# UCSD-Comp-Imaging/Nerf-Simple

Measured on AMD Instinct MI355X. Metric: ray-samples/sec at 800x800x128, higher is better.
Workload: dtype f16

## Files before the change

### nerf-simple_amd/csrc/mlp16_chain.h

```cpp
#pragma once
#include "nerf_device.h"
#include <utility>

typedef elem_t ex8 __attribute__((ext_vector_type(8)));
typedef elem_t ex2 __attribute__((ext_vector_type(2)));

namespace {

using namespace nerf_layout;

constexpr int NCB = 2;
constexpr int WAVES = 16 / NCB;
constexpr int TILE_PTS = WAVES * 16 * NCB;

template <class P>
__host__ __device__ constexpr int layer_chunks(int L) { return (P::mt(L) + P::tpc(L) - 1) / P::tpc(L); }
template <class P>
__host__ __device__ constexpr int chunk_first(int L) {
    int c = 0;
    for (int i = 0; i < L; ++i) c += layer_chunks<P>(i);
    return c;
}
template <class P>
constexpr int NUM_CHUNKS = chunk_first<P>(P::LAYERS);
template <class P>
__host__ __device__ constexpr int chunk_layer(int cc) {
    int L = 0;
    while (cc >= layer_chunks<P>(L)) { cc -= layer_chunks<P>(L); ++L; }
    return L;
}
template <class P>
__host__ __device__ constexpr int chunk_tiles(int cc) {
    const int L = chunk_layer<P>(cc), C = cc - chunk_first<P>(L);
    const int left = P::mt(L) - C * P::tpc(L);
    return left < P::tpc(L) ? left : P::tpc(L);
}
template <class P>
__host__ __device__ constexpr int chunk_kib(int cc) { return chunk_tiles<P>(cc) * b16_ks(chunk_layer<P>(cc)); }
template <class P>
__host__ __device__ constexpr int chunk_off_kib(int cc) {
    const int L = chunk_layer<P>(cc), C = cc - chunk_first<P>(L);
    return P::layer_off_kib(L) + C * P::tpc(L) * b16_ks(L);
}
template <class P>
__host__ __device__ constexpr int tile_mfmas() {
    int m = 0;
    for (int cc = 0; cc < NUM_CHUNKS<P>; ++cc) m += chunk_kib<P>(cc) * NCB;
    return m;
}

constexpr int LDS_WBUF = 40 * 1024;
constexpr int LDS_BIAS = 0;
constexpr int LDS_W0 = 10 * 1024;
constexpr int LDS_CHAIN_END = LDS_W0 + 2 * LDS_WBUF;
static_assert(B16_BIAS_FLOATS * 4 <= LDS_W0, "bias table");
template <class P>
__host__ __device__ constexpr bool plan_fits() {
    for (int cc = 0; cc < NUM_CHUNKS<P>; ++cc)
        if (chunk_kib<P>(cc) * 1024 > LDS_WBUF) return false;
    return NUM_CHUNKS<P> % 2 == 0;
}

struct Ctx {
    __amdgpu_buffer_rsrc_t wrsrc;
    unsigned wave_goff, lane16;
    unsigned b_wread[2];
    unsigned s_wdst[2];
    unsigned b_bias;
    unsigned b_posx, b_posd;
    int wave, lane;
};

struct WFrag {
    ex8 a[4];
    f32x4 bias0;
};

template <bool RELU>
__device__ __forceinline__ unsigned pack2(float a, float b) {
    const f32x2 v = {a, b};
    const ex2 r = __builtin_convertvector(v, ex2);
    if constexpr (RELU) {
        const s16x2 z = {0, 0};
        return __builtin_bit_cast(unsigned, __builtin_elementwise_max(__builtin_bit_cast(s16x2, r), z));
    } else {
        return __builtin_bit_cast(unsigned, r);
    }
}

template <class P, int CC>
using Stage = ChunkDma<Ctx, (CC + 1) % NUM_CHUNKS<P>, chunk_kib<P>((CC + 1) % NUM_CHUNKS<P>), chunk_off_kib<P>((CC + 1) % NUM_CHUNKS<P>), WAVES>;

template <int L, int Q, int SAVE = 0, class St>
__device__ __forceinline__ void epilogue_piece(int i, const f32x4 (&acc)[NCB][2], ex8 (&dst)[NCB][8], St& st) {
    static_assert(!SAVE || St::Plan::SAVE, "this plan has no training forward");
    constexpr LayerDesc D = layer_desc(L);
    const int cb = i >> 2, j2 = i & 3;
    if constexpr (Q == 0 && L >= 1 && L <= 9) {
        if (j2 == 0) st.bad |= __builtin_amdgcn_classf(acc[cb][0][0], 0x207);
    }
    if constexpr (L == 10) {
        if (j2 == 0) { st.rgb[cb][0] = acc[cb][0][0]; st.rgb[cb][1] = acc[cb][0][1]; st.rgb[cb][2] = acc[cb][0][2]; }
    } else if constexpr (L == 8 && Q == 8) {
        if (j2 == 0) st.sigma[cb] = acc[cb][0][0];
    } else {
        u32x4 w = __builtin_bit_cast(u32x4, dst[cb][Q]);
        w[j2] = pack2<D.relu != 0>(acc[cb][j2 >> 1][2 * (j2 & 1)], acc[cb][j2 >> 1][2 * (j2 & 1) + 1]);
        dst[cb][Q] = __builtin_bit_cast(ex8, w);
        if constexpr (SAVE == 2) {
            constexpr int GS = (L & 1) * 2 + ((Q >> 2) & 1);
            st.amax[GS] = f8_absmax<D.relu == 0>(((Q & 3) == 0 && i == 0) ? 0.f : st.amax[GS], acc[cb][j2 >> 1][2 * (j2 & 1)],
                                                 acc[cb][j2 >> 1][2 * (j2 & 1) + 1]);
            if constexpr ((Q & 3) == 3) {
                if (i == 4 * NCB - 1) {
                    static_assert(NCB == 2, "store_group_f8 takes the two column blocks of a wave");
                    constexpr int Q0 = Q - 3;
                    char* tb = st.acts + (f8_offset_bytes(L, st.P) + st.tile * F8_BLOCK_BYTES);
                    char* sp = st.acts + (f8_scale_offset_bytes(L, st.P) + st.tile * 64);
                    const __amdgpu_buffer_rsrc_t rs = __builtin_amdgcn_make_buffer_rsrc(tb, 0, (int)F8_BLOCK_BYTES, 0x00020000);
                    const __amdgpu_buffer_rsrc_t rss = __builtin_amdgcn_make_buffer_rsrc(sp, 0, 64, 0x00020000);
                    const u32x4 g0[4] = {__builtin_bit_cast(u32x4, dst[0][Q0]), __builtin_bit_cast(u32x4, dst[0][Q0 + 1]),
                                         __builtin_bit_cast(u32x4, dst[0][Q0 + 2]), __builtin_bit_cast(u32x4, dst[0][Q0 + 3])};
                    const u32x4 g1[4] = {__builtin_bit_cast(u32x4, dst[1][Q0]), __builtin_bit_cast(u32x4, dst[1][Q0 + 1]),
                                         __builtin_bit_cast(u32x4, dst[1][Q0 + 2]), w};
                    store_group_f8<2>(rs, st.loff[0], Q0 * 8192, rss, (int)(threadIdx.x & 63), (int)(threadIdx.x >> 6) * 8 + Q0,
                                      g0, g1, st.amax[GS]);
                }
            }
        }
        if constexpr (SAVE) {
            if (SAVE == 1 && j2 == 3) {
                char* tb = st.acts + (act_offset_bytes(L, st.P) + st.tile * ACT_BLOCK_BYTES);
                const __amdgpu_buffer_rsrc_t rs = __builtin_amdgcn_make_buffer_rsrc(tb, 0, (int)ACT_BLOCK_BYTES, 0x00020000);
                store_granule<2>(rs, st.loff[cb], Q * 16384, w);
            }
            if constexpr (D.relu != 0) {
                static_assert(NCB == 2, "mask layout: two column blocks per wave");
                const unsigned wj = w[j2];
                unsigned t;
                asm("v_pk_min_u16 %0, %1, %2" : "=v"(t) : "v"(wj), "s"(0x00010001u));
                const int pos = (Q & 3) * 4 + j2;
                st.mb[cb][Q >> 2] = pos == 0 ? t : ((t << pos) | st.mb[cb][Q >> 2]);
                if (pos == 15) {
                    char* mp = st.acts + (st.mask_tile + ((long long)L * mask_tiles(st.P) * 4 + (cb * 2 + (Q >> 2))) * 2048);
                    *reinterpret_cast<unsigned*>(mp + (unsigned)(threadIdx.x * 4)) = st.mb[cb][Q >> 2];
                }
            }
        }
    }
}

template <int SAVE>
__host__ __device__ constexpr int pair_vmem_ops(int L, int Q) {
    if (!SAVE || L < 0 || L == 10 || (L == 8 && Q == 8)) return 0;
    const int masks = (layer_desc(L).relu != 0 && (Q & 3) == 3) ? NCB : 0;
    return (SAVE == 2 ? ((Q & 3) == 3 ? F8_GROUP + 1 : 0) : NCB) + masks;
}
template <int SAVE>
__host__ __device__ constexpr int pair_mask_ops(int L, int Q) {
    if (!SAVE || L < 0 || L == 10 || (L == 8 && Q == 8)) return 0;
    return (layer_desc(L).relu != 0 && (Q & 3) == 3) ? NCB : 0;
}
template <int SAVE>
__host__ __device__ constexpr int vmem_before_barrier(int L, int PL, int PQ, int pair0, int npair_in, int pend_m0, int pend_per,
                                                      int pair_m0, int mt, int m_limit) {
    int n = 0;
    const int last = 4 * NCB - 1;
    if (PL >= 0) {
        const int masks = pair_mask_ops<SAVE>(PL, PQ), data = pair_vmem_ops<SAVE>(PL, PQ) - masks;
        for (int cb = 0; cb < NCB; ++cb) {
            const int own = 4 * cb + 3;
            if (pend_m0 + own / pend_per < m_limit) n += masks / NCB + (SAVE == 2 ? 0 : data / NCB);
        }
        if (SAVE == 2 && pend_m0 + last / pend_per < m_limit) n += data;
    }
    for (int j = 0; j < npair_in; ++j) {
        const int masks = pair_mask_ops<SAVE>(L, pair0 + j), data = pair_vmem_ops<SAVE>(L, pair0 + j) - masks;
        for (int cb = 0; cb < NCB; ++cb) {
            const int own = 4 * cb + 3;
            if (pair_m0 + j * 2 * mt + own < m_limit) n += masks / NCB + (SAVE == 2 ? 0 : data / NCB);
        }
        if (SAVE == 2 && pair_m0 + j * 2 * mt + last < m_limit) n += data;
    }
    return n;
}
template <int L, int P0, int N, int SAVE, int J = 0, class St>
__device__ __forceinline__ void in_chunk_epilogue(int j, int i, const f32x4 (&acc)[NCB][2], ex8 (&dst)[NCB][8], St& st) {
    if constexpr (J < N) {
        if (j == J) epilogue_piece<L, P0 + J, SAVE>(i, acc, dst, st);
        else in_chunk_epilogue<L, P0, N, SAVE, J + 1>(j, i, acc, dst, st);
    }
}

template <int L, int C, int PL, int PQ, int SAVE, class St>
__device__ __forceinline__ void chunk_step(const Ctx& c, St& st, ex8 (&in)[NCB][8], ex8 (&out)[NCB][8]) {
    using P = typename St::Plan;
    constexpr LayerDesc D = layer_desc(L);
    constexpr int KS_CHAIN = D.chain_k / 32;
    constexpr int KS_EXTRA = D.extra_slots / 32;
    constexpr int KS = KS_CHAIN + KS_EXTRA;
    constexpr int CC = chunk_first<P>(L) + C;
    constexpr int NT = chunk_tiles<P>(CC);
    constexpr int RT0 = C * P::tpc(L);
    constexpr int F = NT * KS;
    constexpr int AHEAD = 4;
    constexpr int BIAS_OFF = LDS_BIAS + (P::bias_off(L) + 16 * RT0) * 4;
    constexpr int MT = NCB * KS;
    constexpr int PEND_M0 = (L == 10) ? 0 : (NT * MT >= 4 * NCB + 4 ? 2 : 0);
    constexpr int PEND_PER = (L == 10) ? 2 : 1;
    constexpr int PAIR0 = RT0 / 2;
    constexpr int NPAIR_IN = NT >= 4 ? NT / 2 - 1 : 0;
    constexpr int PAIR_M0 = 2 * MT + (MT >= 4 * NCB + 2 ? 2 : 0);
    static_assert(NT < 4 || NT % 2 == 0, "whole pairs per chunk");
    static_assert(PL < 0 || PL == L || (PL == 8 && PQ == 8) || NCB * PQ >= PEND_M0 + 4 * NCB / PEND_PER,
                  "pending pair finished too late");
    const unsigned wb = c.b_wread[CC & 1];
    constexpr int NCC = (CC + 1) % NUM_CHUNKS<P>;
    constexpr int NL = chunk_layer<P>(NCC);
    constexpr int NF = chunk_tiles<P>(NCC) * (layer_desc(NL).chain_k / 32 + layer_desc(NL).extra_slots / 32);
    constexpr int NBIAS_OFF = LDS_BIAS + (P::bias_off(NL) + 16 * (NCC - chunk_first<P>(NL)) * P::tpc(NL)) * 4;
    const unsigned nwb = c.b_wread[NCC & 1];
    constexpr int TAIL = 3;
    constexpr int FB = F <= TAIL ? F : F - TAIL;
    constexpr int VMEM_N = vmem_before_barrier<SAVE>(L, PL, PQ, PAIR0, NPAIR_IN, PEND_M0, PEND_PER, PAIR_M0, MT, FB * NCB);
    WFrag& wf = *st.wf;
    auto barrier_and_prefetch = [&]() {
        asm volatile("s_waitcnt lgkmcnt(0)" ::: "memory");
        chunk_barrier<VMEM_N>();
#pragma unroll
        for (int f = 0; f < AHEAD && f < NF; ++f) wf.a[f] = lds_load<ex8>(nwb, f * 1024);
        wf.bias0 = lds_load<f32x4>(c.b_bias, NBIAS_OFF);
        __builtin_amdgcn_sched_barrier(0);
    };

    constexpr int SPREAD = 4;
    constexpr bool DMA_SPREAD = !SAVE && 1 + SPREAD * (Stage<P, CC>::PIECES - 1) + 8 <= FB * NCB;
    if constexpr (!DMA_SPREAD) Stage<P, CC>::issue(c);
    __builtin_amdgcn_sched_barrier(0);

    ex8 a[AHEAD];
#pragma unroll
    for (int f = 0; f < AHEAD && f < F; ++f) a[f] = wf.a[f];
    ex8 bx[NCB][KS_EXTRA > 0 ? KS_EXTRA : 1];
    if constexpr (KS_EXTRA > 0) {
#pragma unroll
        for (int cb = 0; cb < NCB; ++cb)
#pragma unroll
            for (int e = 0; e < KS_EXTRA; ++e) {
                if constexpr (D.extra_kind == 1) bx[cb][e] = lds_load<ex8>(c.b_posx, cb * 2048 + e * 1024);
                else bx[cb][e] = lds_load<ex8>(st.posd_off[cb], e * 1024);
            }
    }
    f32x4 acc[NCB][NT];
    acc[0][0] = wf.bias0;
    for (int cb = 1; cb < NCB; ++cb) acc[cb][0] = acc[0][0];
    __builtin_amdgcn_sched_barrier(0);

    ex8 as_prev = a[0];
    f32x4 c_prev = acc[0][0];
#pragma unroll
    for (int t = 0; t < NT; ++t) {
#pragma unroll
        for (int ks = 0; ks < KS; ++ks) {
            const int f = t * KS + ks;
            if (f == FB) barrier_and_prefetch();
            const ex8 as = a[f % AHEAD];
            if (f + AHEAD < F) a[f % AHEAD] = lds_load<ex8>(wb, (f + AHEAD) * 1024);
            if (t + 1 < NT && ks == KS / 2) {
                acc[0][t + 1 < NT ? t + 1 : 0] = lds_load<f32x4>(c.b_bias, BIAS_OFF + 64 * (t + 1));
                for (int cb = 1; cb < NCB; ++cb) acc[cb][t + 1 < NT ? t + 1 : 0] = acc[0][t + 1 < NT ? t + 1 : 0];
            }
            __builtin_amdgcn_sched_barrier(0);
#pragma unroll
            for (int cb = 0; cb < NCB; ++cb) {
                const int m = f * NCB + cb;
                ex8 bs;
                if (ks < KS_CHAIN) bs = in[cb][ks < KS_CHAIN ? ks : 0];
                else bs = bx[cb][KS_EXTRA > 0 ? (ks - KS_CHAIN < KS_EXTRA ? ks - KS_CHAIN : 0) : 0];
                const f32x4 c_old = acc[cb][t];
                acc[cb][t] = NERF_MFMA(as, bs, c_old, 0, 0, 0);
                asm volatile("" :: "v"(c_prev));
                c_prev = c_old;
                if constexpr (DMA_SPREAD) {
                    if (m % SPREAD == 1 && m / SPREAD < Stage<P, CC>::PIECES) Stage<P, CC>::issue_piece(c, m / SPREAD);
                }
                if constexpr (PL >= 0) {
                    if (m >= PEND_M0 && m < PEND_M0 + 4 * NCB / PEND_PER) {
#pragma unroll
                        for (int k = 0; k < PEND_PER; ++k) {
                            const int i = (m - PEND_M0) * PEND_PER + k;
                            if constexpr (PL == L) epilogue_piece<PL, PQ, SAVE>(i, st.pend, out, st);
                            else epilogue_piece<PL, PQ, SAVE>(i, st.pend, in, st);
                        }
                    }
                }
                if constexpr (NPAIR_IN > 0) {
                    const int j = (m - PAIR_M0) / (2 * MT), pm = (m - PAIR_M0) - j * (2 * MT);
                    if (m >= PAIR_M0 && j < NPAIR_IN && pm < 4 * NCB) {
                        f32x4 pr[NCB][2];
                        for (int q_ = 0; q_ < NCB; ++q_) { pr[q_][0] = acc[q_][2 * j]; pr[q_][1] = acc[q_][2 * j + 1]; }
                        in_chunk_epilogue<L, PAIR0, NPAIR_IN, SAVE>(j, pm, pr, out, st);
                    }
                }
                __builtin_amdgcn_sched_barrier(0);
            }
            asm volatile("" :: "v"(as_prev));
            as_prev = as;
            __builtin_amdgcn_sched_barrier(0);
        }
    }
    asm volatile("" :: "v"(as_prev));
    asm volatile("" :: "v"(c_prev));
#pragma unroll
    for (int cb = 0; cb < NCB; ++cb) {
        st.pend[cb][0] = acc[cb][NT >= 2 ? NT - 2 : 0];
        st.pend[cb][1] = acc[cb][NT - 1];
    }
    if constexpr (FB == F) barrier_and_prefetch();
}

__host__ __device__ constexpr int prev_layer(int L, int C) { return C > 0 ? L : L - 1; }
template <class P>
__host__ __device__ constexpr int prev_pair(int L, int C) {
    return C > 0 ? C * P::tpc(L) / 2 - 1 : (L > 0 ? (L - 1 == 8 ? 8 : P::mt(L - 1) / 2 - 1) : 0);
}

template <int L, int SAVE, class St, int... Cs>
__device__ __forceinline__ void run_layer_seq(const Ctx& c, St& st, ex8 (&in)[NCB][8], ex8 (&out)[NCB][8],
                                              std::integer_sequence<int, Cs...>) {
    using P = typename St::Plan;
    (chunk_step<L, Cs, prev_layer(L, Cs), prev_pair<P>(L, Cs), SAVE>(c, st, in, out), ...);
}
template <int L, int SAVE = 0, class St>
__device__ __forceinline__ void run_layer(const Ctx& c, St& st, ex8 (&in)[NCB][8], ex8 (&out)[NCB][8]) {
    run_layer_seq<L, SAVE>(c, st, in, out, std::make_integer_sequence<int, layer_chunks<typename St::Plan>(L)>{});
}

__device__ __forceinline__ void flag_nonfinite(const Ctx& c, bool bad) {
    if (bad) __builtin_amdgcn_raw_buffer_store_b32(1u, c.wrsrc, (int)(B16_STATUS_OFF + 4 * NERF_STATUS_WORD_NONFINITE), 0, 0);
}

}
```

### nerf-simple_amd/csrc/mlp_bwd_16.hip

```cpp
#include "nerf_device.h"
#include "launchers.h"
#include <utility>

using namespace nerf_layout;

typedef __bf16 ex8 __attribute__((ext_vector_type(8)));
typedef __bf16 ex2 __attribute__((ext_vector_type(2)));
typedef unsigned u32x2 __attribute__((ext_vector_type(2)));

struct BwdArgs {
    const float* d_raw;
    const void* image;
    const char* acts;
    char* dys;
    long long P;
    int store_e4m3;
};

namespace {

constexpr int WAVES = 8;
constexpr int TILE_PTS = WAVES * 32;
constexpr int TPC = 4;

__host__ __device__ constexpr int layer_chunks(int b) { return (bwd_mt(b) + TPC - 1) / TPC; }
__host__ __device__ constexpr int chunk_first(int b) {
    int c = 0;
    for (int i = 0; i < b; ++i) c += layer_chunks(i);
    return c;
}
constexpr int NUM_CHUNKS = chunk_first(NUM_BWD);
__host__ __device__ constexpr int chunk_layer(int cc) {
    int b = 0;
    while (cc >= layer_chunks(b)) { cc -= layer_chunks(b); ++b; }
    return b;
}
__host__ __device__ constexpr int chunk_kib(int cc) { return TPC * bwd_ks(chunk_layer(cc)); }
__host__ __device__ constexpr int chunk_off_kib(int cc) {
    const int b = chunk_layer(cc), C = cc - chunk_first(b);
    return bwd_layer_off_kib(b) + C * TPC * bwd_ks(b);
}

constexpr int LDS_WBUF = 40 * 1024;
constexpr int LDS_W0 = 0;
constexpr int LDS_TOTAL = 2 * LDS_WBUF;
static_assert(NUM_CHUNKS % 2 == 0, "buffer parity must repeat per tile");

static_assert(ACT_TILE_PTS == TILE_PTS && MASK_TILE_PTS == TILE_PTS, "activation blocks and mask tiles are the kernel's tiles");

struct Ctx {
    __amdgpu_buffer_rsrc_t wrsrc;
    unsigned wave_goff, lane16;
    unsigned b_wread[2], s_wdst[2];
    int wave, lane;
};

struct State {
    ex8 X[2][8], Y[2][8];
    f32x4 pend[2][2];
    u32x4 mk[2];
    long long mask_tile;
    ex8 bx_rgb[2], bx_sig[2];
    const char* acts;
    char* dys;
    long long P, tile;
    int loff[2];
    float amax[4];
};

__device__ __forceinline__ unsigned pack2(float a, float b) {
    const f32x2 v = {a, b};
    return __builtin_bit_cast(unsigned, __builtin_convertvector(v, ex2));
}

template <int CC>
using Stage = ChunkDma<Ctx, (CC + 1) % NUM_CHUNKS, chunk_kib((CC + 1) % NUM_CHUNKS), chunk_off_kib((CC + 1) % NUM_CHUNKS), WAVES>;

template <int A>
__device__ __forceinline__ void load_mask(const State& st, u32x4& m) {
    const char* mp = st.acts + (st.mask_tile + (long long)A * mask_tiles(st.P) * 8192);
#pragma unroll
    for (int d = 0; d < 4; ++d) m[d] = *reinterpret_cast<const unsigned*>(mp + d * 2048 + (unsigned)(threadIdx.x * 4));
}

template <int B, int Q, bool F8>
__device__ __forceinline__ void epilogue_piece(int i, const f32x4 (&acc)[2][2], ex8 (&dst)[2][8], State& st) {
    constexpr BwdDesc D = bwd_desc(B);
    constexpr int LOUT = 9 - B;
    const int cb = i >> 2, j2 = i & 3;
    float v0 = acc[cb][j2 >> 1][2 * (j2 & 1)], v1 = acc[cb][j2 >> 1][2 * (j2 & 1) + 1];
    if constexpr (D.mask_act >= 0) {
        const unsigned mw = st.mk[B & 1][cb * 2 + (Q >> 2)];
        const int pos = (Q & 3) * 4 + j2;
        v0 = __builtin_bit_cast(float, __builtin_bit_cast(int, v0) & ((int)(mw << (31 - pos)) >> 31));
        v1 = __builtin_bit_cast(float, __builtin_bit_cast(int, v1) & ((int)(mw << (15 - pos)) >> 31));
    }
    u32x4 w = __builtin_bit_cast(u32x4, dst[cb][Q]);
    w[j2] = pack2(v0, v1);
    dst[cb][Q] = __builtin_bit_cast(ex8, w);
    if constexpr (F8) {
        constexpr int GS = (B & 1) * 2 + ((Q >> 2) & 1);
        st.amax[GS] = f8_absmax<true>(((Q & 3) == 0 && i == 0) ? 0.f : st.amax[GS], v0, v1);
        if constexpr ((Q & 3) == 3) {
            if (i == 7) {
                constexpr int Q0 = Q - 3;
                char* tb = st.dys + (f8_offset_bytes(LOUT, st.P) + st.tile * F8_BLOCK_BYTES);
                char* sp = st.dys + (f8_scale_offset_bytes(LOUT, st.P) + st.tile * 64);
                const __amdgpu_buffer_rsrc_t rs = __builtin_amdgcn_make_buffer_rsrc(tb, 0, (int)F8_BLOCK_BYTES, 0x00020000);
                const __amdgpu_buffer_rsrc_t rss = __builtin_amdgcn_make_buffer_rsrc(sp, 0, 64, 0x00020000);
                const u32x4 g0[4] = {__builtin_bit_cast(u32x4, dst[0][Q0]), __builtin_bit_cast(u32x4, dst[0][Q0 + 1]),
                                     __builtin_bit_cast(u32x4, dst[0][Q0 + 2]), __builtin_bit_cast(u32x4, dst[0][Q0 + 3])};
                const u32x4 g1[4] = {__builtin_bit_cast(u32x4, dst[1][Q0]), __builtin_bit_cast(u32x4, dst[1][Q0 + 1]),
                                     __builtin_bit_cast(u32x4, dst[1][Q0 + 2]), w};
                store_group_f8<2>(rs, st.loff[0], Q0 * 8192, rss, (int)(threadIdx.x & 63), (int)(threadIdx.x >> 6) * 8 + Q0, g0, g1,
                                  st.amax[GS]);
            }
        }
    } else if (j2 == 3) {
        char* tb = st.dys + (act_offset_bytes(LOUT, st.P) + st.tile * ACT_BLOCK_BYTES);
        const __amdgpu_buffer_rsrc_t rs = __builtin_amdgcn_make_buffer_rsrc(tb, 0, (int)ACT_BLOCK_BYTES, 0x00020000);
        store_granule<2>(rs, st.loff[cb], Q * 16384, w);
    }
}

template <int B, int C, int PB, int PQ, bool F8>
__device__ __forceinline__ void chunk_step(const Ctx& c, State& st, ex8 (&in)[2][8], ex8 (&out)[2][8]) {
    constexpr BwdDesc D = bwd_desc(B);
    constexpr int KS_CHAIN = D.chain_k / 32;
    constexpr int KS = KS_CHAIN + D.extra;
    constexpr int CC = chunk_first(B) + C;
    constexpr int NT = TPC;
    constexpr int F = NT * KS;
    constexpr int AHEAD = 4;
    constexpr int MT = 2 * KS;
    constexpr int TOTAL_M = NT * MT;
    constexpr bool PEND_EARLY = TOTAL_M < 24 || (PB != B && PB >= 0 && 2 * PQ < 12);
    constexpr int PEND_PER = PEND_EARLY ? 2 : 1;
    constexpr int PEND_M0 = PEND_EARLY ? 0 : 2;
    static_assert(PB < 0 || PB == B || 2 * PQ >= PEND_M0 + 8 / PEND_PER, "pending pair finished too late");
    constexpr int PAIR_M0 = TOTAL_M >= 24 ? 2 * MT + 2 : 2 * MT;
    constexpr int PAIR_PER = (TOTAL_M - PAIR_M0) >= 8 ? 1 : 2;
    const unsigned wb = c.b_wread[CC & 1];
    static_assert(bwd_mt(B) % TPC == 0, "row tiles per backward layer");

    Stage<CC>::issue(c);
    __builtin_amdgcn_sched_barrier(0);

    ex8 a[AHEAD];
#pragma unroll
    for (int f = 0; f < AHEAD && f < F; ++f) a[f] = lds_load<ex8>(wb, f * 1024);
    if constexpr (C == 1 && B + 1 < NUM_BWD) {
        if constexpr (bwd_desc(B + 1).mask_act >= 0) load_mask<bwd_desc(B + 1).mask_act>(st, st.mk[(B + 1) & 1]);
    }
    static_assert(layer_chunks(B) >= 2, "the mask prefetch lives in chunk 1");
    f32x4 acc[2][NT];
#pragma unroll
    for (int cb = 0; cb < 2; ++cb)
#pragma unroll
        for (int t = 0; t < NT; ++t) acc[cb][t] = f32x4{0.f, 0.f, 0.f, 0.f};
    __builtin_amdgcn_sched_barrier(0);

    ex8 as_prev = a[0];
    f32x4 c_prev = acc[0][0];
#pragma unroll
    for (int t = 0; t < NT; ++t) {
#pragma unroll
        for (int ks = 0; ks < KS; ++ks) {
            const int f = t * KS + ks;
            const ex8 as = a[f % AHEAD];
            if (f + AHEAD < F) a[f % AHEAD] = lds_load<ex8>(wb, (f + AHEAD) * 1024);
            __builtin_amdgcn_sched_barrier(0);
#pragma unroll
            for (int cb = 0; cb < 2; ++cb) {
                const int m = f * 2 + cb;
                ex8 bs;
                if (ks < KS_CHAIN) bs = in[cb][ks < KS_CHAIN ? ks : 0];
                else bs = (B == 0) ? st.bx_rgb[cb] : st.bx_sig[cb];
                const f32x4 c_old = acc[cb][t];
                acc[cb][t] = __builtin_amdgcn_mfma_f32_16x16x32_bf16(as, bs, c_old, 0, 0, 0);
                asm volatile("" :: "v"(c_prev));
                c_prev = c_old;
                if constexpr (PB >= 0) {
                    if (m >= PEND_M0 && m < PEND_M0 + 8 / PEND_PER) {
#pragma unroll
                        for (int k = 0; k < PEND_PER; ++k) {
                            const int i = (m - PEND_M0) * PEND_PER + k;
                            if constexpr (PB == B) epilogue_piece<PB, PQ, F8>(i, st.pend, out, st);
                            else epilogue_piece<PB, PQ, F8>(i, st.pend, in, st);
                        }
                    }
                }
                if (m >= PAIR_M0 && m < PAIR_M0 + 8 / PAIR_PER) {
                    const f32x4 pr[2][2] = {{acc[0][0], acc[0][1]}, {acc[1][0], acc[1][1]}};
#pragma unroll
                    for (int k = 0; k < PAIR_PER; ++k)
                        epilogue_piece<B, 2 * C, F8>((m - PAIR_M0) * PAIR_PER + k, pr, out, st);
                }
                __builtin_amdgcn_sched_barrier(0);
            }
            asm volatile("" :: "v"(as_prev));
            as_prev = as;
            __builtin_amdgcn_sched_barrier(0);
        }
    }
    asm volatile("" :: "v"(as_prev));
    asm volatile("" :: "v"(c_prev));
#pragma unroll
    for (int cb = 0; cb < 2; ++cb) {
        st.pend[cb][0] = acc[cb][NT - 2];
        st.pend[cb][1] = acc[cb][NT - 1];
    }
    constexpr bool PREFETCH = C == 1 && B + 1 < NUM_BWD && bwd_desc(B + 1 < NUM_BWD ? B + 1 : B).mask_act >= 0;
    constexpr int STORES = F8 ? ((PB >= 0 && (PQ & 3) == 3) ? F8_GROUP + 1 : 0) : (PB >= 0 ? 2 : 0) + 2;
    static_assert(!F8 || ((2 * C) & 3) != 3, "an in-chunk pair never ends a group");
    chunk_barrier<STORES + (PREFETCH ? 4 : 0)>();
}

__host__ __device__ constexpr int prev_layer(int b, int C) { return C > 0 ? b : b - 1; }
__host__ __device__ constexpr int prev_pair(int b, int C) {
    return C > 0 ? 2 * C - 1 : (b > 0 ? bwd_mt(b - 1) / 2 - 1 : 0);
}
template <int B, bool F8, int... Cs>
__device__ __forceinline__ void run_layer_seq(const Ctx& c, State& st, ex8 (&in)[2][8], ex8 (&out)[2][8],
                                              std::integer_sequence<int, Cs...>) {
    (chunk_step<B, Cs, prev_layer(B, Cs), prev_pair(B, Cs), F8>(c, st, in, out), ...);
}
template <int B, bool F8>
__device__ __forceinline__ void run_layer(const Ctx& c, State& st, ex8 (&in)[2][8], ex8 (&out)[2][8]) {
    run_layer_seq<B, F8>(c, st, in, out, std::make_integer_sequence<int, layer_chunks(B)>{});
}

template <bool F8>
__device__ __forceinline__ void bwd_body(const BwdArgs& a, long long ntiles) {
    Ctx c;
    c.wave = __builtin_amdgcn_readfirstlane(threadIdx.x >> 6);
    c.lane = threadIdx.x & 63;
    c.wrsrc = __builtin_amdgcn_make_buffer_rsrc(const_cast<void*>(a.image), 0, (int)BWD_IMAGE_BYTES, 0x00020000);
    c.wave_goff = c.wave * 1024;
    c.lane16 = c.lane * 16;
#pragma unroll
    for (int p = 0; p < 2; ++p) {
        c.b_wread[p] = LDS_W0 + p * LDS_WBUF + c.lane * 16;
        c.s_wdst[p] = LDS_W0 + p * LDS_WBUF + c.wave * 1024;
    }
    Stage<NUM_CHUNKS - 1>::issue(c);
    asm volatile("s_waitcnt vmcnt(0)" ::: "memory");
    __syncthreads();

    const int col = c.lane & 15, g = c.lane >> 4;
    for (long long tile = blockIdx.x; tile < ntiles; tile += gridDim.x) {
        const long long tile_base = tile * TILE_PTS;
        asm volatile("" : "+s"(c.wave_goff));
        State st;
        st.acts = a.acts;
        st.dys = a.dys;
        st.P = a.P;
        st.mask_tile = F8 ? f8_mask_offset_bytes(0, tile, 0, a.P) : mask_offset_bytes(0, tile, 0, a.P);
        st.tile = tile;
        load_mask<bwd_desc(0).mask_act>(st, st.mk[0]);
        const __bf16 z = (__bf16)0.f;
#pragma unroll
        for (int cb = 0; cb < 2; ++cb) {
            const long long p = tile_base + c.wave * 32 + cb * 16 + col;
            st.loff[cb] = p < a.P ? block_lane_offset(g, c.wave * 32 + cb * 16 + col) : LOFF_INVALID;
            if (F8 && cb == 0)
                st.loff[0] = tile_base + c.wave * 32 + 16 * (c.lane >> 5) + col < a.P ? f8_lane_offset(c.lane, c.wave) : LOFF_INVALID;
            f32x4 d = {0.f, 0.f, 0.f, 0.f};
            if (p < a.P) d = *reinterpret_cast<const f32x4*>(a.d_raw + p * 4);
            const bool g0 = g == 0;
            st.bx_rgb[cb] = ex8{g0 ? (__bf16)d[0] : z, g0 ? (__bf16)d[1] : z, g0 ? (__bf16)d[2] : z, z, z, z, z, z};
            st.bx_sig[cb] = ex8{g0 ? (__bf16)d[3] : z, z, z, z, z, z, z, z};
        }
        run_layer<0, F8>(c, st, st.X, st.X);
        run_layer<1, F8>(c, st, st.X, st.Y);
        run_layer<2, F8>(c, st, st.Y, st.X);
        run_layer<3, F8>(c, st, st.X, st.Y);
        run_layer<4, F8>(c, st, st.Y, st.X);
        run_layer<5, F8>(c, st, st.X, st.Y);
        run_layer<6, F8>(c, st, st.Y, st.X);
        run_layer<7, F8>(c, st, st.X, st.Y);
        run_layer<8, F8>(c, st, st.Y, st.X);
        run_layer<9, F8>(c, st, st.X, st.Y);
#pragma unroll
        for (int i = 0; i < 8; ++i) epilogue_piece<9, bwd_mt(9) / 2 - 1, F8>(i, st.pend, st.Y, st);
    }
}

__global__ __launch_bounds__(WAVES * 64, WAVES / 4) void nerf_mlp_bwd_kernel(BwdArgs a, long long ntiles) {
    extern __shared__ __attribute__((aligned(16))) char smem[];
    (void)smem;
    bwd_body<false>(a, ntiles);
}
__global__ __launch_bounds__(WAVES * 64, WAVES / 4) void nerf_mlp_bwd_e4m3_kernel(BwdArgs a, long long ntiles) {
    extern __shared__ __attribute__((aligned(16))) char smem[];
    (void)smem;
    bwd_body<true>(a, ntiles);
}

}

extern "C" int nerf_amd_launch_mlp_backward(const float* d_raw, const void* image, const void* acts, void* dys,
                                            long long P, int store_e4m3, hipStream_t stream) {
    (void)hipGetLastError();
    if (P <= 0) return 0;
    BwdArgs a{d_raw, image, reinterpret_cast<const char*>(acts), reinterpret_cast<char*>(dys), P, store_e4m3};
    const long long ntiles = (P + TILE_PTS - 1) / TILE_PTS;
    const int cus = device_cus();
    const long long grid = ntiles < cus ? ntiles : cus;
    auto kern = store_e4m3 ? nerf_mlp_bwd_e4m3_kernel : nerf_mlp_bwd_kernel;
    const hipError_t e = allow_dynamic_lds(reinterpret_cast<const void*>(kern), LDS_TOTAL);
    if (e != hipSuccess) return (int)e;
    hipLaunchKernelGGL(kern, dim3((unsigned)grid), dim3(WAVES * 64), LDS_TOTAL, stream, a, ntiles);
    return (int)hipGetLastError();
}
```

### nerf-simple_amd/csrc/nerf_device.h

```cpp
#pragma once
#include <hip/hip_runtime.h>
#include <stdint.h>
#include <atomic>
#include "nerf_layout.h"

typedef __bf16 bf16x8 __attribute__((ext_vector_type(8)));
typedef __bf16 bf16x2 __attribute__((ext_vector_type(2)));
typedef short s16x2 __attribute__((ext_vector_type(2)));
typedef unsigned short u16x2 __attribute__((ext_vector_type(2)));
typedef float f32x2 __attribute__((ext_vector_type(2)));
typedef float f32x4 __attribute__((ext_vector_type(4)));
typedef float f32x16 __attribute__((ext_vector_type(16)));
typedef unsigned u32x4 __attribute__((ext_vector_type(4)));

#define NERF_FLAG_TS_GIVEN 1u
#define NERF_FLAG_DEVICE_RNG 2u
#define NERF_FLAG_SEED_IN_MEMORY 4u
#define NERF_FLAG_STORE_E4M3 8u

struct MlpArgs {
    const float* pts;
    const float* rays;
    const float* u;
    const float* tbins;
    const void* packed;
    float* raw;
    float* ts_out;
    void* acts;
    long long P;
    long long ray_id0;
    unsigned long long seed;
    int N;
    unsigned flags;
    float* rgb;
    float* disp;
    float* alpha;
    float* acc;
    float* w;
    float* pixels;
};

struct DensityArgs {
    const float* pts;
    long long stride;
    const void* packed;
    float* sigma;
    long long P;
    long long ny, nz;
    float lo[3], step[3];
};

constexpr int NERF_MAX_DEVICES = 64;
inline int device_cus() {
    static int cache[NERF_MAX_DEVICES] = {};
    int dev = 0;
    if (hipGetDevice(&dev) != hipSuccess || dev < 0 || dev >= NERF_MAX_DEVICES) return 256;
    if (cache[dev] == 0) {
        int cus = 256;
        if (hipDeviceGetAttribute(&cus, hipDeviceAttributeMultiprocessorCount, dev) != hipSuccess || cus <= 0) cus = 256;
        cache[dev] = cus;
    }
    return cache[dev];
}
inline hipError_t allow_dynamic_lds(const void* kernel, int bytes) {
    struct Slot { const void* kernel; int dev; };
    static Slot slots[128];
    static std::atomic<int> used{0};
    int dev = 0;
    if (hipGetDevice(&dev) != hipSuccess) dev = -1;
    const int n = used.load(std::memory_order_acquire);
    for (int i = 0; i < n && i < 128; ++i)
        if (slots[i].kernel == kernel && slots[i].dev == dev) return hipSuccess;
    const hipError_t e = hipFuncSetAttribute(kernel, hipFuncAttributeMaxDynamicSharedMemorySize, bytes);
    if (e == hipSuccess && dev >= 0) {
        const int i = used.load(std::memory_order_relaxed);
        if (i < 128) {
            slots[i] = Slot{kernel, dev};
            used.store(i + 1, std::memory_order_release);
        }
    }
    return e;
}

constexpr int LOFF_INVALID = 0x40000000;
__host__ __device__ constexpr int swapped_chunk(int g) { return (g & 1) * 2 + (g >> 1); }
__host__ __device__ constexpr int block_lane_offset(int g, int local) { return swapped_chunk(g) * 4096 + local * 16; }

template <int AUX = 0>
__device__ __forceinline__ void store_granule(__amdgpu_buffer_rsrc_t rs, int voffset, int soffset, u32x4 w) {
    const auto s0 = __builtin_amdgcn_permlane16_swap(w[0], w[2], false, false);
    const auto s1 = __builtin_amdgcn_permlane16_swap(w[1], w[3], false, false);
    const unsigned o0 = s0[0], o1 = s1[0], o2 = s0[1], o3 = s1[1];
    __builtin_amdgcn_raw_buffer_store_b128(u32x4{o0, o1, o2, o3}, rs, voffset, soffset, AUX);
    asm volatile("s_nop 1" ::"v"(o0), "v"(o1), "v"(o2), "v"(o3) : "memory");
}

template <bool ABS>
__device__ __forceinline__ float f8_absmax(float running, float v0, float v1) {
    float r;
    if constexpr (ABS) asm("v_max3_f32 %0, %1, |%2|, |%3|" : "=v"(r) : "v"(running), "v"(v0), "v"(v1));
    else asm("v_max3_f32 %0, %1, %2, %3" : "=v"(r) : "v"(running), "v"(v0), "v"(v1));
    return r;
}
__device__ __forceinline__ int f8_wave_max_exponent(float m) {
    int r;
    asm volatile("s_nop 1\n\t"
                 "v_max_f32_dpp %1, %1, %1 quad_perm:[1,0,3,2] row_mask:0xf bank_mask:0xf\n\ts_nop 1\n\t"
                 "v_max_f32_dpp %1, %1, %1 quad_perm:[2,3,0,1] row_mask:0xf bank_mask:0xf\n\ts_nop 1\n\t"
                 "v_max_f32_dpp %1, %1, %1 row_half_mirror row_mask:0xf bank_mask:0xf\n\ts_nop 1\n\t"
                 "v_max_f32_dpp %1, %1, %1 row_mirror row_mask:0xf bank_mask:0xf\n\ts_nop 1\n\t"
                 "v_max_f32_dpp %1, %1, %1 row_bcast:15 row_mask:0xa bank_mask:0xf\n\ts_nop 1\n\t"
                 "v_max_f32_dpp %1, %1, %1 row_bcast:31 row_mask:0xc bank_mask:0xf\n\ts_nop 1\n\t"
                 "v_readlane_b32 %0, %1, 63"
                 : "=s"(r), "+v"(m));
    return (r >> 23) & 0xff;
}
__device__ __forceinline__ unsigned f8_cvt4(unsigned lo, unsigned hi, float scale) {
    unsigned r;
    asm("v_cvt_scalef32_pk_fp8_bf16 %0, %1, %3\n\tv_cvt_scalef32_pk_fp8_bf16 %0, %2, %3 op_sel:[0,0,1]"
        : "=&v"(r) : "v"(lo), "v"(hi), "s"(scale));
    return r;
}
__host__ __device__ constexpr int f8_lane_offset(int lane, int wave) {
    return ((lane >> 4) & 1) * 4096 + (wave * 32 + 16 * (lane >> 5) + (lane & 15)) * 16;
}
template <int AUX = 0>
__device__ __forceinline__ void store_fragment_f8(__amdgpu_buffer_rsrc_t rs_data, int voff, int soff_data, u32x4 w0, u32x4 w1,
                                                  float scale) {
    const unsigned a0 = f8_cvt4(w0[0], w0[1], scale), b0 = f8_cvt4(w0[2], w0[3], scale);
    unsigned a1 = f8_cvt4(w1[0], w1[1], scale), b1 = f8_cvt4(w1[2], w1[3], scale);
    asm volatile("s_nop 1" : "+v"(a1), "+v"(b1));
    const auto x0 = __builtin_amdgcn_permlane32_swap(a0, a1, false, false);
    const auto x1 = __builtin_amdgcn_permlane32_swap(b0, b1, false, false);
    const auto y0 = __builtin_amdgcn_permlane16_swap(x0[0], x1[0], false, false);
    const auto y1 = __builtin_amdgcn_permlane16_swap(x0[1], x1[1], false, false);
    const unsigned o0 = y0[0], o1 = y0[1], o2 = y1[0], o3 = y1[1];
#if defined(F8_TIMING) && F8_TIMING == 2
    asm volatile("" ::"v"(o0), "v"(o1), "v"(o2), "v"(o3));
#else
    __builtin_amdgcn_raw_buffer_store_b128(u32x4{o0, o1, o2, o3}, rs_data, voff, soff_data,
#if defined(F8_TIMING) && F8_TIMING == 3
                                           0);
#else
                                           AUX);
#endif
    asm volatile("s_nop 1" ::"v"(o0), "v"(o1), "v"(o2), "v"(o3) : "memory");
#endif
}
constexpr int F8_GROUP = 4;
template <int AUX = 0>
__device__ __forceinline__ void store_group_f8(__amdgpu_buffer_rsrc_t rs_data, int voff, int soff_data,
                                               __amdgpu_buffer_rsrc_t rs_scale, int lane, int scale_byte,
                                               const u32x4 (&w0)[F8_GROUP], const u32x4 (&w1)[F8_GROUP], float amax) {
#if defined(F8_TIMING) && F8_TIMING == 1
    const int e = (__builtin_bit_cast(int, amax) >> 23) & 0xff;
#else
    const int e = f8_wave_max_exponent(amax);
#endif
    const int sb = e > 8 ? e - 7 : 1;
    const float scale = __builtin_bit_cast(float, sb << 23);
#pragma unroll
    for (int k = 0; k < F8_GROUP; ++k) store_fragment_f8<AUX>(rs_data, voff, soff_data + k * 8192, w0[k], w1[k], scale);
#if !(defined(F8_TIMING) && F8_TIMING == 2)
    __builtin_amdgcn_raw_buffer_store_b32((unsigned)sb * 0x01010101u, rs_scale, lane == 0 ? scale_byte : LOFF_INVALID, 0, 0);
#endif
}

template <int N>
__device__ __forceinline__ void chunk_barrier() {
    asm volatile("s_waitcnt vmcnt(%0)" ::"n"(N) : "memory");
    __builtin_amdgcn_s_barrier();
    asm volatile("" ::: "memory");
}

__device__ __forceinline__ void wave_lds_fence() {
    __builtin_amdgcn_s_waitcnt(0xc07f);
    __builtin_amdgcn_wave_barrier();
}

typedef __attribute__((address_space(3))) char lds_char;
typedef __attribute__((address_space(3))) void lds_void;
template <class T>
__device__ __forceinline__ T lds_load(unsigned base, int imm) {
    return *reinterpret_cast<const __attribute__((address_space(3))) T*>(reinterpret_cast<lds_char*>(0) + base + imm);
}
template <class T>
__device__ __forceinline__ void lds_store(unsigned base, int imm, const T& v) {
    *reinterpret_cast<__attribute__((address_space(3))) T*>(reinterpret_cast<lds_char*>(0) + base + imm) = v;
}

template <class C, int NEXT, int KIB, int OFF_KIB, int WAVES>
struct ChunkDma {
    static constexpr int PIECES = (KIB + WAVES - 1) / WAVES;
    static constexpr int SRC_OFF = OFF_KIB * 1024;
    static __device__ __forceinline__ void issue_piece(const C& c, int p) {
        __builtin_amdgcn_raw_ptr_buffer_load_lds(
            c.wrsrc, reinterpret_cast<lds_void*>(reinterpret_cast<lds_char*>(0) + c.s_wdst[NEXT & 1] + p * (WAVES * 1024)), 16,
            c.lane16, c.wave_goff + (SRC_OFF + p * WAVES * 1024), 0, 0);
    }
    static __device__ __forceinline__ void issue(const C& c) {
#pragma unroll
        for (int p = 0; p < PIECES; ++p) issue_piece(c, p);
    }
};

__device__ __forceinline__ unsigned philox_word(unsigned long long seed, unsigned long long ctr) {
    unsigned c0 = (unsigned)ctr, c1 = (unsigned)(ctr >> 32), c2 = 0x6e657266u, c3 = 0x616d6421u;
    unsigned k0 = (unsigned)seed, k1 = (unsigned)(seed >> 32);
#pragma unroll
    for (int r = 0; r < 10; ++r) {
        const unsigned long long p0 = 0xD2511F53ull * c0, p1 = 0xCD9E8D57ull * c2;
        const unsigned n0 = (unsigned)(p1 >> 32) ^ c1 ^ k0, n2 = (unsigned)(p0 >> 32) ^ c3 ^ k1;
        c1 = (unsigned)p1; c3 = (unsigned)p0; c0 = n0; c2 = n2;
        k0 += 0x9E3779B9u; k1 += 0xBB67AE85u;
    }
    return c0;
}
__device__ __forceinline__ float philox_uniform(unsigned long long seed, unsigned long long ctr) {
    return (float)(philox_word(seed, ctr) >> 8) * (1.0f / 16777216.0f);
}

__device__ __forceinline__ float mul_rn(float a, float b) {
#pragma clang fp contract(off)
    return a * b;
}
__device__ __forceinline__ float add_rn(float a, float b) {
#pragma clang fp contract(off)
    return a + b;
}
__device__ __forceinline__ float sub_rn(float a, float b) {
#pragma clang fp contract(off)
    return a - b;
}
__device__ __forceinline__ float sqrt_rn(float a) { return sqrtf(a); }

__device__ __forceinline__ float norm3(float x, float y, float z) {
    return sqrt_rn(__fmaf_rn(z, z, __fmaf_rn(y, y, mul_rn(x, x))));
}

struct PointIn {
    float x, y, z, d1, d2, d3, t;
};

struct RaySample { long long b; int i; };
__device__ __forceinline__ RaySample split_point(long long b0, int r0, int local, int N) {
    const unsigned tt = (unsigned)(r0 + local);
    unsigned q = (unsigned)((float)tt * __frcp_rn((float)N));
    if ((long long)q * N > (long long)tt) --q;
    if ((long long)(q + 1) * N <= (long long)tt) ++q;
    return RaySample{b0 + q, (int)(tt - q * (unsigned)N)};
}
__device__ __forceinline__ RaySample split_point(long long p, int N) {
    const long long b = p / N;
    return RaySample{b, (int)(p - b * N)};
}

__device__ __forceinline__ unsigned long long effective_seed(const MlpArgs& a) {
    if (!(a.flags & NERF_FLAG_SEED_IN_MEMORY)) return a.seed;
    const unsigned long long v = *reinterpret_cast<const unsigned long long*>(a.u);
    const unsigned lo = __builtin_amdgcn_readfirstlane((unsigned)v), hi = __builtin_amdgcn_readfirstlane((unsigned)(v >> 32));
    return a.seed + (((unsigned long long)hi << 32) | lo);
}

__device__ __forceinline__ float device_rng_uniform(const MlpArgs& a, RaySample rs) {
    unsigned long long seed = effective_seed(a);
    asm volatile("" : "+s"(seed));
    return philox_uniform(seed, (unsigned long long)((a.ray_id0 + rs.b) * a.N + rs.i));
}

template <bool DIR = true>
__device__ __forceinline__ PointIn fetch_point_rays(const MlpArgs& a, long long p, RaySample rs, float u_pre = 0.f,
                                                    bool have_u = false) {
    PointIn r;
    const long long b = rs.b;
    const int i = rs.i;
    const float* ray = a.rays + b * 6;
    const float ox = ray[0], oy = ray[1], oz = ray[2];
    const float dx = ray[3], dy = ray[4], dz = ray[5];
    float t;
    if (a.flags & NERF_FLAG_TS_GIVEN) {
        t = __builtin_nontemporal_load(a.u + p);
    } else {
        float u;
        if (a.flags & NERF_FLAG_DEVICE_RNG)
            u = have_u ? u_pre : philox_uniform(effective_seed(a), (unsigned long long)((a.ray_id0 + b) * a.N + i));
        else
            u = __builtin_nontemporal_load(a.u + p);
        const float bin_diff = sub_rn(a.tbins[1], a.tbins[0]);
        t = add_rn(mul_rn(bin_diff, u), a.tbins[i]);
    }
    r.t = t;
    r.x = add_rn(ox, mul_rn(dx, t));
    r.y = add_rn(oy, mul_rn(dy, t));
    r.z = add_rn(oz, mul_rn(dz, t));
    if constexpr (DIR) {
        const float nrm = norm3(dx, dy, dz);
        r.d1 = __fdiv_rn(dx, nrm);
        r.d2 = __fdiv_rn(dy, nrm);
        r.d3 = __fdiv_rn(dz, nrm);
    } else {
        r.d1 = r.d2 = r.d3 = 0.f;
    }
    return r;
}

__device__ __forceinline__ PointIn fetch_point_rays(const MlpArgs& a, long long p) {
    return fetch_point_rays(a, p, split_point(p, a.N));
}

__device__ __forceinline__ PointIn fetch_point_pts(const MlpArgs& a, long long p) {
    PointIn r;
    const float* v = a.pts + p * 6;
    r.x = v[0]; r.y = v[1]; r.z = v[2];
    r.d1 = v[3]; r.d2 = v[4]; r.d3 = v[5];
    r.t = 0.f;
    return r;
}

struct TwoF { float hi, lo; };
__device__ __forceinline__ TwoF to_revolutions(float x) {
    const float C_HI = 0.15915494f;
    const float C_LO = 6.4206382e-09f;
    x = __builtin_amdgcn_fmed3f(x, -0x1p100f, 0x1p100f);
    TwoF q;
    q.hi = mul_rn(x, C_HI);
    const float err = __fmaf_rn(x, C_HI, -q.hi);
    q.lo = __fmaf_rn(x, C_LO, err);
    return q;
}
__device__ __forceinline__ float enc_lane(TwoF q, int idx) {
    const float sc = __builtin_amdgcn_ldexpf(1.0f, idx >> 1);
    const float fr = __builtin_amdgcn_fractf(q.hi * sc) + q.lo * sc + ((idx & 1) ? 0.25f : 0.f);
    return __builtin_amdgcn_sinf(fr);
}
__device__ __forceinline__ void sincos_rev_fast(TwoF q, float scale, float& s, float& c) {
    const float f = __builtin_amdgcn_fractf(q.hi * scale) + q.lo * scale;
    s = __builtin_amdgcn_sinf(f);
    c = __builtin_amdgcn_cosf(f);
}
```

Before: 1.400 billion.

## Move backward chunk barrier before tail and prefetch next chunk's weight fragments

The backward MLP kernel now places the per-chunk barrier a few fragment steps before the end of the chunk and issues the next chunk's first LDS weight-fragment reads immediately after it. The fragments are carried across chunks through a persistent WFrag register struct, so the next chunk's wait on LDS latency is hidden. The change also splits the permlane16 swap of the granule store so half of it happens earlier, switches the non-f8 ReLU mask to a packed 16-bit operation, and staggers the forward pass's mask-bit accumulation by one step. In exchange, register pressure goes up from the persistent fragments, and the vmem counts given to the barrier become more intricate and error-prone.

```diff
diff --git a/nerf-simple_amd/csrc/mlp16_chain.h b/nerf-simple_amd/csrc/mlp16_chain.h
--- a/nerf-simple_amd/csrc/mlp16_chain.h
+++ b/nerf-simple_amd/csrc/mlp16_chain.h
@@ -129,18 +129,27 @@
             }
         }
         if constexpr (SAVE) {
+            if constexpr (D.relu != 0) {
+                static_assert(NCB == 2, "mask layout: two column blocks per wave");
+                auto take_bits = [&](int jj) {
+                    const unsigned wj = w[jj];
+                    unsigned t;
+                    asm("v_pk_min_u16 %0, %1, %2" : "=v"(t) : "v"(wj), "s"(0x00010001u));
+                    const int p = (Q & 3) * 4 + jj;
+                    unsigned m = p == 0 ? t : ((t << p) | st.mb[cb][Q >> 2]);
+                    asm("" : "+v"(m));
+                    st.mb[cb][Q >> 2] = m;
+                };
+                if (j2 >= 1) take_bits(j2 - 1);
+                if (j2 == 3) take_bits(3);
+            }
             if (SAVE == 1 && j2 == 3) {
                 char* tb = st.acts + (act_offset_bytes(L, st.P) + st.tile * ACT_BLOCK_BYTES);
                 const __amdgpu_buffer_rsrc_t rs = __builtin_amdgcn_make_buffer_rsrc(tb, 0, (int)ACT_BLOCK_BYTES, 0x00020000);
                 store_granule<2>(rs, st.loff[cb], Q * 16384, w);
             }
             if constexpr (D.relu != 0) {
-                static_assert(NCB == 2, "mask layout: two column blocks per wave");
-                const unsigned wj = w[j2];
-                unsigned t;
-                asm("v_pk_min_u16 %0, %1, %2" : "=v"(t) : "v"(wj), "s"(0x00010001u));
                 const int pos = (Q & 3) * 4 + j2;
-                st.mb[cb][Q >> 2] = pos == 0 ? t : ((t << pos) | st.mb[cb][Q >> 2]);
                 if (pos == 15) {
                     char* mp = st.acts + (st.mask_tile + ((long long)L * mask_tiles(st.P) * 4 + (cb * 2 + (Q >> 2))) * 2048);
                     *reinterpret_cast<unsigned*>(mp + (unsigned)(threadIdx.x * 4)) = st.mb[cb][Q >> 2];
diff --git a/nerf-simple_amd/csrc/mlp_bwd_16.hip b/nerf-simple_amd/csrc/mlp_bwd_16.hip
--- a/nerf-simple_amd/csrc/mlp_bwd_16.hip
+++ b/nerf-simple_amd/csrc/mlp_bwd_16.hip
@@ -55,7 +55,12 @@
     int wave, lane;
 };
 
+struct WFrag {
+    ex8 a[4];
+};
+
 struct State {
+    WFrag* wf;
     ex8 X[2][8], Y[2][8];
     f32x4 pend[2][2];
     u32x4 mk[2];
@@ -89,14 +94,28 @@
     constexpr int LOUT = 9 - B;
     const int cb = i >> 2, j2 = i & 3;
     float v0 = acc[cb][j2 >> 1][2 * (j2 & 1)], v1 = acc[cb][j2 >> 1][2 * (j2 & 1) + 1];
-    if constexpr (D.mask_act >= 0) {
-        const unsigned mw = st.mk[B & 1][cb * 2 + (Q >> 2)];
-        const int pos = (Q & 3) * 4 + j2;
-        v0 = __builtin_bit_cast(float, __builtin_bit_cast(int, v0) & ((int)(mw << (31 - pos)) >> 31));
-        v1 = __builtin_bit_cast(float, __builtin_bit_cast(int, v1) & ((int)(mw << (15 - pos)) >> 31));
+    const unsigned mw = D.mask_act >= 0 ? st.mk[B & 1][cb * 2 + (Q >> 2)] : 0u;
+    const int pos = (Q & 3) * 4 + j2;
+    if constexpr (D.mask_act >= 0 && F8) {
+        int m0 = (int)(mw << (31 - pos)) >> 31, m1 = (int)(mw << (15 - pos)) >> 31;
+        asm("" : "+v"(m0));
+        asm("" : "+v"(m1));
+        v0 = __builtin_bit_cast(float, __builtin_bit_cast(int, v0) & m0);
+        v1 = __builtin_bit_cast(float, __builtin_bit_cast(int, v1) & m1);
+    }
+    u32x2_t s0 = {0u, 0u};
+    if (!F8 && j2 == 3) {
+        const u32x4 wd = __builtin_bit_cast(u32x4, dst[cb][Q]);
+        s0 = granule_trade(wd[0], wd[2]);
+    }
+    unsigned pk = pack2(v0, v1);
+    if constexpr (D.mask_act >= 0 && !F8) {
+        const u16x2 up = __builtin_bit_cast(u16x2, mw) << (unsigned short)(15 - pos);
+        const s16x2 keep = __builtin_bit_cast(s16x2, up) >> (short)15;
+        pk &= __builtin_bit_cast(unsigned, keep);
     }
     u32x4 w = __builtin_bit_cast(u32x4, dst[cb][Q]);
-    w[j2] = pack2(v0, v1);
+    w[j2] = pk;
     dst[cb][Q] = __builtin_bit_cast(ex8, w);
     if constexpr (F8) {
         constexpr int GS = (B & 1) * 2 + ((Q >> 2) & 1);
@@ -119,8 +138,16 @@
     } else if (j2 == 3) {
         char* tb = st.dys + (act_offset_bytes(LOUT, st.P) + st.tile * ACT_BLOCK_BYTES);
         const __amdgpu_buffer_rsrc_t rs = __builtin_amdgcn_make_buffer_rsrc(tb, 0, (int)ACT_BLOCK_BYTES, 0x00020000);
-        store_granule<2>(rs, st.loff[cb], Q * 16384, w);
-    }
+        store_granule<2>(rs, st.loff[cb], Q * 16384, s0, granule_trade(w[1], w[3]));
+    }
+}
+
+template <bool F8>
+__host__ __device__ constexpr int stores_before(int m0, int per, int m_limit, bool ends_group) {
+    int n = 0;
+    for (int piece = 3; piece < 8; piece += 4)
+        if (m0 + piece / per < m_limit) n += F8 ? (piece == 7 && ends_group ? F8_GROUP + 1 : 0) : 1;
+    return n;
 }
 
 template <int B, int C, int PB, int PQ, bool F8>
@@ -142,13 +169,32 @@
     constexpr int PAIR_PER = (TOTAL_M - PAIR_M0) >= 8 ? 1 : 2;
     const unsigned wb = c.b_wread[CC & 1];
     static_assert(bwd_mt(B) % TPC == 0, "row tiles per backward layer");
+    constexpr int NCC = (CC + 1) % NUM_CHUNKS;
+    constexpr int NF = TPC * bwd_ks(chunk_layer(NCC));
+    const unsigned nwb = c.b_wread[NCC & 1];
+    constexpr int TAIL = 3;
+    constexpr int FB = F - TAIL;
+    static_assert(F > TAIL && AHEAD > TAIL && NF >= AHEAD, "every fragment read of the chunk is issued in front of its barrier");
+    constexpr bool PREFETCH = C == 1 && B + 1 < NUM_BWD && bwd_desc(B + 1 < NUM_BWD ? B + 1 : B).mask_act >= 0;
+    static_assert(!F8 || ((2 * C) & 3) != 3, "an in-chunk pair never ends a group");
+    constexpr int VMEM_N = (PREFETCH ? 4 : 0) +
+                           (PB >= 0 ? stores_before<F8>(PEND_M0, PEND_PER, 2 * FB, (PQ & 3) == 3) : 0) +
+                           stores_before<F8>(PAIR_M0, PAIR_PER, 2 * FB, false);
+    WFrag& wf = *st.wf;
+    auto barrier_and_prefetch = [&]() {
+        asm volatile("s_waitcnt lgkmcnt(0)" ::: "memory");
+        chunk_barrier<VMEM_N>();
+#pragma unroll
+        for (int f = 0; f < AHEAD; ++f) wf.a[f] = lds_load<ex8>(nwb, f * 1024);
+        __builtin_amdgcn_sched_barrier(0);
+    };
 
     Stage<CC>::issue(c);
     __builtin_amdgcn_sched_barrier(0);
 
     ex8 a[AHEAD];
 #pragma unroll
-    for (int f = 0; f < AHEAD && f < F; ++f) a[f] = lds_load<ex8>(wb, f * 1024);
+    for (int f = 0; f < AHEAD; ++f) a[f] = wf.a[f];
     if constexpr (C == 1 && B + 1 < NUM_BWD) {
         if constexpr (bwd_desc(B + 1).mask_act >= 0) load_mask<bwd_desc(B + 1).mask_act>(st, st.mk[(B + 1) & 1]);
     }
@@ -167,6 +213,7 @@
 #pragma unroll
         for (int ks = 0; ks < KS; ++ks) {
             const int f = t * KS + ks;
+            if (f == FB) barrier_and_prefetch();
             const ex8 as = a[f % AHEAD];
             if (f + AHEAD < F) a[f % AHEAD] = lds_load<ex8>(wb, (f + AHEAD) * 1024);
             __builtin_amdgcn_sched_barrier(0);
@@ -210,10 +257,6 @@
         st.pend[cb][0] = acc[cb][NT - 2];
         st.pend[cb][1] = acc[cb][NT - 1];
     }
-    constexpr bool PREFETCH = C == 1 && B + 1 < NUM_BWD && bwd_desc(B + 1 < NUM_BWD ? B + 1 : B).mask_act >= 0;
-    constexpr int STORES = F8 ? ((PB >= 0 && (PQ & 3) == 3) ? F8_GROUP + 1 : 0) : (PB >= 0 ? 2 : 0) + 2;
-    static_assert(!F8 || ((2 * C) & 3) != 3, "an in-chunk pair never ends a group");
-    chunk_barrier<STORES + (PREFETCH ? 4 : 0)>();
 }
 
 __host__ __device__ constexpr int prev_layer(int b, int C) { return C > 0 ? b : b - 1; }
@@ -246,12 +289,16 @@
     Stage<NUM_CHUNKS - 1>::issue(c);
     asm volatile("s_waitcnt vmcnt(0)" ::: "memory");
     __syncthreads();
+    WFrag wf;
+#pragma unroll
+    for (int f = 0; f < 4; ++f) wf.a[f] = lds_load<ex8>(c.b_wread[0], f * 1024);
 
     const int col = c.lane & 15, g = c.lane >> 4;
     for (long long tile = blockIdx.x; tile < ntiles; tile += gridDim.x) {
         const long long tile_base = tile * TILE_PTS;
         asm volatile("" : "+s"(c.wave_goff));
         State st;
+        st.wf = &wf;
         st.acts = a.acts;
         st.dys = a.dys;
         st.P = a.P;
diff --git a/nerf-simple_amd/csrc/nerf_device.h b/nerf-simple_amd/csrc/nerf_device.h
--- a/nerf-simple_amd/csrc/nerf_device.h
+++ b/nerf-simple_amd/csrc/nerf_device.h
@@ -86,13 +86,20 @@
 __host__ __device__ constexpr int swapped_chunk(int g) { return (g & 1) * 2 + (g >> 1); }
 __host__ __device__ constexpr int block_lane_offset(int g, int local) { return swapped_chunk(g) * 4096 + local * 16; }
 
+typedef unsigned u32x2_t __attribute__((ext_vector_type(2)));
+__device__ __forceinline__ u32x2_t granule_trade(unsigned a, unsigned b) {
+    const auto s = __builtin_amdgcn_permlane16_swap(a, b, false, false);
+    return u32x2_t{s[0], s[1]};
+}
 template <int AUX = 0>
-__device__ __forceinline__ void store_granule(__amdgpu_buffer_rsrc_t rs, int voffset, int soffset, u32x4 w) {
-    const auto s0 = __builtin_amdgcn_permlane16_swap(w[0], w[2], false, false);
-    const auto s1 = __builtin_amdgcn_permlane16_swap(w[1], w[3], false, false);
+__device__ __forceinline__ void store_granule(__amdgpu_buffer_rsrc_t rs, int voffset, int soffset, u32x2_t s0, u32x2_t s1) {
     const unsigned o0 = s0[0], o1 = s1[0], o2 = s0[1], o3 = s1[1];
     __builtin_amdgcn_raw_buffer_store_b128(u32x4{o0, o1, o2, o3}, rs, voffset, soffset, AUX);
     asm volatile("s_nop 1" ::"v"(o0), "v"(o1), "v"(o2), "v"(o3) : "memory");
+}
+template <int AUX = 0>
+__device__ __forceinline__ void store_granule(__amdgpu_buffer_rsrc_t rs, int voffset, int soffset, u32x4 w) {
+    store_granule<AUX>(rs, voffset, soffset, granule_trade(w[0], w[2]), granule_trade(w[1], w[3]));
 }
 
 template <bool ABS>
```

Result: no change. 1.399 billion (-0.0%).
